# andreaskoepf/faster-rcnn.torch

Hardware: AMD Instinct MI355X
Metric: images/sec (vgg_small 800x450 fwd+bwd) (higher is better)
Workload: dtype f32 (conv / Linear(13824,1024) operands as 2 x fp16 split planes: 22 significand bits, 3 MFMA partial products; fp32 accumulate)

## Files before the change

### faster-rcnn.torch_amd/csrc/conv.hip

```cpp
#include <cstdlib>

#include "kernels.h"
#include "amax.h"
#include <type_traits>

namespace frcnn {

typedef float f32x16 __attribute__((ext_vector_type(16)));

int conv_cc(int k) { return k == 1 ? 32 : (k == 3 ? 8 : 2); }
int conv_mpad(int M) { return M <= 64 ? 64 : cdiv(M, 128) * 128; }
size_t conv_pack_floats(int Kchan, int M, int k) {
  int cc = conv_cc(k);
  return (size_t)cdiv(Kchan, cc) * cc * k * k * conv_mpad(M);
}

__global__ void pack_weights_kernel(const float* __restrict__ w, int O, int C, int k, int mode,
                                    int Kchan_pad, int M, int Mpad, float* __restrict__ dst) {
  long total = (long)Kchan_pad * k * k * Mpad;
  for (long t = (long)blockIdx.x * blockDim.x + threadIdx.x; t < total;
       t += (long)gridDim.x * blockDim.x) {
    int m = (int)(t % Mpad);
    long row = t / Mpad;
    int h = (int)(row & 1);
// ... 1198 lines not shown
  hipLaunchKernelGGL(wgrad_reduce_map_kernel, dim3(rgrid), dim3(256), 0, s, slab, nSplit, taps, O, C, gw, map);
  return FRCNN_OK;
}

size_t conv_wgrad_workspace_bytes(int Cin, int H, int W, int O, int k, int pad) {
  if (k == 3 && Cin % 64 == 0 && O % 64 == 0) {
    WgradArgs b;
    b.Cin = Cin; b.H = H; b.W = W; b.O = O; b.pad = pad; b.Ho = H + 2 * pad - k + 1; b.Wo = W + 2 * pad - k + 1;
    wgrad_plan(b, k);
    return std::max((size_t)b.nSplit * k * k * O * Cin * 4 + 256, conv_wgradx_workspace_bytes(Cin, H, W, O, pad));
  }
  WgradArgs a;
  a.Cin = Cin; a.H = H; a.W = W; a.O = O; a.pad = pad;
  a.Ho = H + 2 * pad - k + 1; a.Wo = W + 2 * pad - k + 1;
  wgrad_plan(a, k);
  return (size_t)a.nSplit * (k * k * O * Cin + O + 1) * 4 + 256;
}

template <int KS, int TYS, int PM>
static int launch_wgrad_pm(WgradArgs& a, int klass, double flops, float* gw, hipStream_t s) {
  size_t lds = ((size_t)64 * WG_NTP + (size_t)64 * (PM == 2 ? 129 : WG_PP)) * 4;
  static bool attr_set = false;
  if (!attr_set) {
    FR_HIP(hipFuncSetAttribute(reinterpret_cast<const void*>(conv_wgrad_kernel<KS, TYS, PM>),
                               hipFuncAttributeMaxDynamicSharedMemorySize, 160 * 1024));
    attr_set = true;
  }
  int grid = a.oTiles * a.cTiles * a.kyGroups * a.nSplit;
  double bytes = 4.0 * ((double)a.Cin * a.H * a.W + (double)a.O * a.Ho * a.Wo);
  if (frcnn::prof_enabled(klass)) frcnn::prof_before(klass, s);
  hipLaunchKernelGGL((conv_wgrad_kernel<KS, TYS, PM>), dim3(grid), dim3(256), lds, s, a);
// ... 99 lines not shown
```

### faster-rcnn.torch_amd/csrc/net.cpp

```cpp
#include <array>
#include <vector>
#include <cmath>
#include <cstring>

#include "kernels.h"

namespace frcnn {

static const int HEAD_OUT = 18;
static const int SPARSE_MAX_POS = 512;

struct DevBuf {
  void* p = nullptr;
  size_t bytes = 0;
  bool owned = true;
  void view(void* ptr, size_t n) { p = ptr; bytes = n; owned = false; }
  int ensure(size_t need) {
    if (need <= bytes) return FRCNN_OK;
    if (p && owned) (void)hipFree(p);
    owned = true;
    p = nullptr; bytes = 0;
    FR_HIP(hipMalloc(&p, need + 64));
    bytes = need;
    return FRCNN_OK;
// ... 13 lines not shown
  DevBuf x, gx;
  int am = -1;
};

struct Block {
  int first_conv, nconv;
  bool has_drop;
  float p_drop;
  DevBuf scale;
  DevBuf pooled, gpooled;
  DevBuf pidx;
  int Hp, Wp;
  int am = -1;
  bool dc_on = false;
  int nk = 0, nkM = 0, nkK = 0;
  const int* dc_idx = nullptr;
  DevBuf dc_bias;
};

struct Head {
  Conv c3;
  Conv c1;
  int input;
  DevBuf delta;
  const int* sp_pos = nullptr;
  int sp_count = -1;
  DevBuf spD, spHX, spHY, spGH, spCol, spDX;
  DevBuf spOut, spSlab;
  hipStream_t stream = nullptr;
  hipEvent_t done = nullptr;
// ... 11 lines not shown
  DevBuf xp, xpT, gp, gpT;
  int x_form = 0;
  DevBuf am;
  const float* am_w_of = nullptr;
  long am_w_gen = -1;
};

}

using namespace frcnn;

static int g_drop_compact = -1;
static int drop_compact_on() {
  if (g_drop_compact < 0) g_drop_compact = getenv("FRCNN_DROP_COMPACT") ? (atoi(getenv("FRCNN_DROP_COMPACT")) != 0) : 1;
  return g_drop_compact;
}
static int pool_stream(int slot, hipStream_t* out) {
  static hipStream_t pool[8] = {};
  if (!pool[slot]) FR_HIP(hipStreamCreateWithFlags(&pool[slot], hipStreamNonBlocking));
  *out = pool[slot];
  return FRCNN_OK;
}

static int g_sparse_heads = -1;
static int sparse_heads_on() {
  if (g_sparse_heads < 0) g_sparse_heads = getenv("FRCNN_SPARSE_HEADS") ? (atoi(getenv("FRCNN_SPARSE_HEADS")) != 0) : 1;
  return g_sparse_heads;
}
static int g_static_weights = 0;
static long g_static_gen = 0;
// ... 550 lines not shown
int frcnn_model_update_join(frcnn_model* m, void* stream) {
  FR_CHECK(m != nullptr, "model_update_join: null model");
  FR_TRY(ensure_update_stream(m));
  FR_HIP(hipEventRecord(m->upd_join_ev, m->cw));
  FR_HIP(hipStreamWaitEvent(S(stream), m->upd_join_ev, 0));
  return FRCNN_OK;
}

int frcnn_get_option(const char* name, int* value) {
  FR_CHECK(name != nullptr && value != nullptr, "get_option: null argument");
  if (strcmp(name, "side_stream") == 0) { *value = side_enabled() ? 1 : 0; return FRCNN_OK; }
  if (strcmp(name, "gemm_x_roles") == 0) { *value = get_gemm_x_roles(); return FRCNN_OK; }
  if (strcmp(name, "deterministic") == 0) { *value = deterministic() ? 1 : 0; return FRCNN_OK; }
  if (strcmp(name, "static_weights") == 0) { *value = g_static_weights; return FRCNN_OK; }
  if (strcmp(name, "drop_compact") == 0) { *value = drop_compact_on(); return FRCNN_OK; }
  if (strcmp(name, "sparse_heads") == 0) { *value = sparse_heads_on(); return FRCNN_OK; }
  if (strcmp(name, "winograd") == 0) { *value = 0; return FRCNN_OK; }
  if (strcmp(name, "cnet_wgrad_async") == 0) { *value = g_cnet_wgrad_async; return FRCNN_OK; }
  if (strcmp(name, "split_bf16") == 0) { *value = get_split_bf16(); return FRCNN_OK; }
  if (strcmp(name, "x3_f16") == 0) { *value = get_x3_f16(); return FRCNN_OK; }
  FR_CHECK(false, "get_option: unknown option '%s'", name);
  return FRCNN_OK;
}

int frcnn_set_option(const char* name, int value) {
  FR_CHECK(name != nullptr, "set_option: null name");
  if (strcmp(name, "side_stream") == 0) { g_side_stream = value ? 1 : 0; return FRCNN_OK; }
  if (strcmp(name, "deterministic") == 0) { set_deterministic(value != 0); return FRCNN_OK; }
  if (strcmp(name, "static_weights") == 0) { g_static_weights = value != 0; ++g_static_gen; return FRCNN_OK; }
  if (strcmp(name, "drop_compact") == 0) { g_drop_compact = value != 0; return FRCNN_OK; }
  if (strcmp(name, "sparse_heads") == 0) { g_sparse_heads = value != 0; return FRCNN_OK; }
  if (strcmp(name, "gemm_x_roles") == 0) { set_gemm_x_roles(value); return FRCNN_OK; }
  if (strcmp(name, "split_bf16") == 0) { set_split_bf16(value); return FRCNN_OK; }
  if (strcmp(name, "x3_f16") == 0) { set_x3_f16(value); return FRCNN_OK; }
  if (strcmp(name, "winograd") == 0) return FRCNN_OK;
  if (strcmp(name, "cnet_wgrad_async") == 0) { g_cnet_wgrad_async = value ? 1 : 0; return FRCNN_OK; }
  FR_CHECK(false, "set_option: unknown option '%s'", name);
  return FRCNN_OK;
}

static int ensure_head_streams(frcnn_model* m);
static int ensure_side(frcnn_model* m) {
  if (!m->side) {
    FR_TRY(pool_stream(0, &m->side));
    FR_HIP(hipEventCreateWithFlags(&m->join_ev, hipEventDisableTiming));
// ... 111 lines not shown
      for (int i = 0; i < C; ++i) keep[i] = frcnn_keep_mask(seed * 131 + b, (unsigned long long)i, blk.p_drop);
    }
    int nk = 0;
    bool binary = true;
    for (int i = 0; i < C; ++i) {
      if (keep[i] == 1.0f) idx_host[my + nk++] = i;
      else if (keep[i] != 0.0f) binary = false;
    }
    if (!binary) continue;
    for (int i = nk; i < C; ++i) idx_host[my + i] = -1;
    const int nkM = std::min(C, (nk + 63) / 64 * 64), nkK = std::min(C, (nk + 15) / 16 * 16);
    if (nk == 0 || nkK >= C) continue;
    if (!conv_x3_eligible(c0.Cin, nkM, 3) || !conv_x3_eligible(nkK, c1.Cout, 3) || !conv_x3_eligible(c1.Cout, nkM, 3) ||
        (b > 0 && !conv_x3_eligible(nkK, c0.Cin, 3)) || !conv_wgradx_eligible(nkM, c1.Cout, 3) || !conv_wgradx_eligible(c0.Cin, nkM, 3))
      continue;
    blk.dc_on = true; blk.nk = nk; blk.nkM = nkM; blk.nkK = nkK; blk.dc_idx = idx_dev + my;
  }
  return FRCNN_OK;
}

static int pack_compact(frcnn_model* m, const float* w, bool f16, hipStream_t s) {
  const unsigned slot = m->dc_step % frcnn_model::DC_RING;
  ++m->dc_step;
  char* hslot = m->dc_pin + (size_t)slot * m->dc_slot_bytes;
  char* dslot = (char*)m->dc_dev.p + (size_t)slot * m->dc_slot_bytes;
  const std::vector<PackXJob>& src = f16 ? m->x3_host16 : m->x3_host;
  PackXJob* jobs = (PackXJob*)hslot;
  int n = 0;
  for (int i = 0; i < (int)src.size(); ++i) {
    PackXJob j = src[i];
    const int ci = m->x3_conv[i];
// ... 687 lines not shown
                            grad + c.b_off, grad + c.a_off, s, (c.x_d && m->f16_packed) ? m->rec(c.am + 1) : nullptr));
      }
      const float* in; const float* in_slope = nullptr; const float* in_scale = nullptr;
      if (st > 0) {
        Conv& pc = m->convs[blk.first_conv + st - 1];
        in = pc.x.f(); in_slope = w + pc.a_off;
        in_scale = (st - 1 == 0 && blk.has_drop) ? blk.scale.f() : nullptr;
      } else {
        in = b == 0 ? m->img.f() : m->blocks[b - 1].pooled.f();
      }
      const bool dc = blk.dc_on && st <= 1;
      int wg_cin = c.Cin, wg_o = c.Cout;
      WgradMap wmap;
      if (dc) {
        wmap.Cfull = c.Cin;
        if (st == 1) { wg_cin = blk.nkM; wmap.cmap = blk.dc_idx; in_scale = nullptr; }
        else { wg_o = blk.nkM; wmap.omap = blk.dc_idx; }
      }
      const float* wa_in = nullptr; const float* wa_g = nullptr;
      if (m->f16_packed && c.x_f && c.x_d && (st > 0 || b > 0)) {
        wa_in = st > 0 ? m->rec(m->convs[blk.first_conv + st - 1].am) : m->rec(m->blocks[b - 1].am);
        wa_g = m->rec(c.am + 1);
      }
      const bool on_caller = use_side && b == 0 && st == 0;
      if (use_side && !on_caller) FR_TRY(fork_side(m, s, n_fork++));
      if (on_caller) {
        FR_TRY(conv_wgrad(in, wg_cin, c.H, c.W, in_slope, in_scale, c.gx.f(), wg_o, c.k, c.pad, grad + c.w_off, m->wg_ws_first.p,
                          m->wg_ws_first.bytes, s, fused_here ? grad + c.b_off : nullptr, wa_in, wa_g, dc ? &wmap : nullptr));
        FR_HIP(hipEventRecord(m->join_ev, ws));
        FR_HIP(hipStreamWaitEvent(s, m->join_ev, 0));
      } else {
// ... 287 lines not shown
```

### faster-rcnn.torch_amd/csrc/wgradx.hip

```cpp
#include <cstdlib>

#include "kernels.h"
#include "amax.h"
#include <type_traits>

namespace frcnn {

typedef float f32x16 __attribute__((ext_vector_type(16)));
typedef __bf16 bf16x8 __attribute__((ext_vector_type(8)));
typedef __bf16 bf16x4 __attribute__((ext_vector_type(4)));
typedef __bf16 bf16x2 __attribute__((ext_vector_type(2)));
typedef float f32x2 __attribute__((ext_vector_type(2)));
typedef _Float16 f16x8 __attribute__((ext_vector_type(8)));
typedef _Float16 f16x2 __attribute__((ext_vector_type(2)));

#define WX_TH 4
#define WX_TW 16
#define WX_GROW 128
#define WX_GPLANE (64 * WX_GROW)
#define WX_XROW 48
#define WX_XCH (6 * WX_XROW)
#define WX_XPLANE (64 * WX_XCH + 8 * 16)
#define WX_LDS (3 * WX_GPLANE + 3 * WX_XPLANE)

bool conv_wgradx_eligible(int Cin, int O, int k) {
  return get_split_bf16() && k == 3 && Cin % 64 == 0 && O % 64 == 0;
}

__device__ __forceinline__ unsigned wx_cvt2(float a, float b) {
  f32x2 v = {a, b};
  bf16x2 r = __builtin_convertvector(v, bf16x2);
  return __builtin_bit_cast(unsigned, r);
}
__device__ __forceinline__ void wx_split4(const float* v, uint2& H, uint2& Mi, uint2& L) {
  unsigned h[2], m[2], l[2];
#pragma unroll
  for (int j = 0; j < 2; ++j) {
    const float x0 = v[2 * j], x1 = v[2 * j + 1];
    h[j] = wx_cvt2(x0, x1);
    const float r0 = x0 - __builtin_bit_cast(float, h[j] << 16), r1 = x1 - __builtin_bit_cast(float, h[j] & 0xFFFF0000u);
    m[j] = wx_cvt2(r0, r1);
// ... 16 lines not shown
}
__device__ __forceinline__ float wx_pow2(int e) { return __builtin_bit_cast(float, (unsigned)(e + 127) << 23); }

struct WgradXArgs {
  const float* in;
  const float* in_slope;
  const float* in_scale;
  const float* g;
  float* slab;
  float* gbias;
  const float* amax_in;
  const float* amax_g;
  const int* omap;
  int Cin, H, W, O, Ho, Wo, pad;
  int tilesX, tilesY, oTiles, cTiles, nSplit;
};

__device__ __forceinline__ unsigned wx_xaddr(int c) { return (unsigned)(c * WX_XCH + (c >> 3) * 16); }
__device__ __forceinline__ unsigned wx_gswz(int o) { const unsigned u = (o >> 1) & 7; return ((u & 3) << 1) | (u >> 2); }

typedef unsigned u32x4 __attribute__((ext_vector_type(4)));
typedef float f32x4u __attribute__((ext_vector_type(4), aligned(4)));

#define WX_PIN(x) asm volatile("" : "+v"(x))

template <int N, class F>
__device__ __forceinline__ void static_for(F&& f) {
  if constexpr (N > 0) {
    static_for<N - 1>(f);
    f(std::integral_constant<int, N - 1>{});
  }
}

template <bool SLOPE, bool SCALE, int VEC, int NP = 3>
__global__ __launch_bounds__(256, 1) void conv_wgradx_kernel(WgradXArgs p) {
  extern __shared__ __attribute__((aligned(16))) char smem[];
  constexpr unsigned LDSI = NP * (WX_GPLANE + WX_XPLANE), XB = NP * WX_GPLANE;
  const int tid = threadIdx.x, lane = tid & 63;
  const int wave = __builtin_amdgcn_readfirstlane(tid >> 6);
  const int wo = wave >> 1, wc = wave & 1;
  const int h = lane >> 5, li = lane & 31;

  int bid;
  {
    const int nblk = gridDim.x, xcd = blockIdx.x & 7, idx = blockIdx.x >> 3;
    const int q = nblk >> 3, r = nblk & 7;
    bid = xcd * q + min(xcd, r) + idx;
  }
  const int ot = bid % p.oTiles; bid /= p.oTiles;
  const int ct = bid % p.cTiles;
  const int split = bid / p.cTiles;
  const int o0 = ot * 64, c0 = ct * 64;
  const int HW = p.H * p.W, HoWo = p.Ho * p.Wo;
  const float slope = SLOPE ? *p.in_slope : 1.f;
  float gmul = 1.f, xmul = 1.f, out_mul = 1.f, out_mul2 = 1.f;
  if (NP == 2) {
    const float ag = amax_load_block(p.amax_g);
    float ax = amax_load_block(p.amax_in);
    if (SLOPE) ax *= fmaxf(1.f, fabsf(slope));
    const int eg = wx_exp(ag, 14), ex = wx_exp(ax, SCALE ? 13 : 14);
    gmul = wx_pow2(eg); xmul = wx_pow2(ex);
    const int et = -(eg + ex), e1 = et / 2;
    out_mul = wx_pow2(e1); out_mul2 = wx_pow2(et - e1);
  }

  f32x16 acc[9];
#pragma unroll
  for (int t = 0; t < 9; ++t)
#pragma unroll
    for (int r = 0; r < 16; ++r) acc[t][r] = 0.f;

  const int srow = tid >> 2, sq = tid & 3;
  const float* const gsrc = p.g + (size_t)(o0 + srow) * HoWo;
  const float* const xsrc = p.in + (size_t)(c0 + srow) * HW;
  auto gat = [&](int elem_off) { return gsrc + elem_off; };
  auto xat = [&](int elem_off) { return xsrc + elem_off; };
  const float xscale = SCALE ? p.in_scale[c0 + srow] : 1.f;
  const unsigned gdst = (unsigned)(srow * WX_GROW) + ((((unsigned)sq >> 1) ^ wx_gswz(srow)) << 4) + (sq & 1) * 8;
  const unsigned xdst = XB + wx_xaddr(srow) + sq * 8;
  int xr[9], xs[9];
#pragma unroll
  for (int k = 0; k < 9; ++k) {
    const int j = sq + 4 * k;
    xr[k] = j / 6; xs[k] = j - 6 * xr[k];
  }

  const int oA = wo * 32 + li, cB = wc * 32 + li;
  const unsigned abase = (unsigned)(oA * WX_GROW) + (((unsigned)h ^ wx_gswz(oA)) << 4);
  const unsigned bbase = XB + wx_xaddr(cB) + h * 16;

  const int nPix = p.tilesX * p.tilesY;
  const int nT = (nPix - split + p.nSplit - 1) / p.nSplit;
  struct Pre {
    float vg[4][4], vx[9][4];
    bool ok[13];
    int oy0, ox0;
  };
#ifdef WX_ONE_SET
  Pre pre[1];
#else
  Pre pre[2];
#endif
  float sr[13][4];
  unsigned sh[13][2], sm[13][2], sl[13][2];
  float bsum = 0.f;
  bool bsum_on = true;
  auto up_lo = [](unsigned v) { return __builtin_bit_cast(float, v << 16); };
  auto up_hi = [](unsigned v) { return __builtin_bit_cast(float, v & 0xFFFF0000u); };
  const int adv_y = p.nSplit / p.tilesX, adv_x = p.nSplit % p.tilesX;
  int w_ty = split / p.tilesX, w_tx = split % p.tilesX, w_i = 0;
  auto load_origin = [&](Pre& P) {
    P.oy0 = w_ty * WX_TH; P.ox0 = w_tx * WX_TW;
    const int more = w_i + 1 < nT ? 1 : 0;
    w_tx += more * adv_x; w_ty += more * adv_y;
    const int wrap = w_tx >= p.tilesX ? 1 : 0;
    w_tx -= wrap * p.tilesX; w_ty += wrap;
    ++w_i;
  };
  auto load_step = [&](auto itc, Pre& P) {
    constexpr int it = decltype(itc)::value;
    const int oy0 = P.oy0, ox0 = P.ox0;
    if constexpr (it < 4) {
      constexpr int k = it;
      const int oy = oy0 + k, ox = ox0 + 4 * sq;
      if (VEC) {
        P.ok[it] = oy < p.Ho && ox < p.Wo;
        const f32x4u v = *reinterpret_cast<const f32x4u*>(gat((oy * p.Wo + ox) & -(int)P.ok[it]));
        P.vg[k][0] = v[0]; P.vg[k][1] = v[1]; P.vg[k][2] = v[2]; P.vg[k][3] = v[3];
      } else {
#pragma unroll
        for (int e = 0; e < 4; ++e) P.vg[k][e] = *gat((oy * p.Wo + ox + e) & -(int)(oy < p.Ho && ox + e < p.Wo));
      }
    } else {
      constexpr int k = it - 4;
      const int iy = oy0 - p.pad + xr[k], ix = ox0 - p.pad - 3 + 4 * xs[k];
      if (VEC) {
        P.ok[it] = (unsigned)iy < (unsigned)p.H && (unsigned)ix < (unsigned)p.W;
        const f32x4u v = *reinterpret_cast<const f32x4u*>(xat((iy * p.W + ix) & -(int)P.ok[it]));
        P.vx[k][0] = v[0]; P.vx[k][1] = v[1]; P.vx[k][2] = v[2]; P.vx[k][3] = v[3];
      } else {
#pragma unroll
        for (int e = 0; e < 4; ++e)
          P.vx[k][e] = *xat((iy * p.W + ix + e) & -(int)((unsigned)iy < (unsigned)p.H && (unsigned)(ix + e) < (unsigned)p.W));
      }
    }
  };
  auto inside = [&](auto itc, int e, Pre& P) -> bool {
    constexpr int it = decltype(itc)::value;
    if (VEC == 1) return P.ok[it];
    if (VEC == 2) {
      if constexpr (it < 4) return P.ok[it] && P.ox0 + 4 * sq + e < p.Wo;
      else return P.ok[it] && P.ox0 - p.pad - 3 + 4 * xs[it < 4 ? 0 : it - 4] + e < p.W;
    }
    if constexpr (it < 4) return P.oy0 + it < p.Ho && P.ox0 + 4 * sq + e < p.Wo;
    else return (unsigned)(P.oy0 - p.pad + xr[it < 4 ? 0 : it - 4]) < (unsigned)p.H &&
                (unsigned)(P.ox0 - p.pad - 3 + 4 * xs[it < 4 ? 0 : it - 4] + e) < (unsigned)p.W;
  };
  constexpr int XPH0 = (SLOPE || SCALE) ? 0 : 4;
  auto stage_step = [&](auto itc, auto phc, unsigned gwb, unsigned xwb, Pre& P) {
    constexpr int it = decltype(itc)::value, ph = decltype(phc)::value;
    if constexpr (ph < 4) {
      constexpr int k = it - 4;
      {
        constexpr int e = ph;
        float v = P.vx[k][e];
        if (SLOPE) v = v > 0.f ? v : slope * v;
        if (SCALE) v *= xscale;
        P.vx[k][e] = inside(itc, e, P) ? v : 0.f;
        WX_PIN(P.vx[k][e]);
      }
    } else if constexpr (ph == 4 || ph == 6) {
      constexpr int j = (ph - 4) / 2;
      float x0 = it < 4 ? P.vg[it < 4 ? it : 0][2 * j] : P.vx[it < 4 ? 0 : it - 4][2 * j];
      float x1 = it < 4 ? P.vg[it < 4 ? it : 0][2 * j + 1] : P.vx[it < 4 ? 0 : it - 4][2 * j + 1];
      if (it < 4 || XPH0 == 4) {
        x0 = inside(itc, 2 * j, P) ? x0 : 0.f;
        x1 = inside(itc, 2 * j + 1, P) ? x1 : 0.f;
      }
      if (it < 4) bsum += bsum_on ? x0 + x1 : 0.f;
      if constexpr (NP == 2) {
        const float mul = it < 4 ? gmul : xmul;
        x0 *= mul; x1 *= mul;
        sh[it][j] = wx_cvt2h(x0, x1);
        const f16x2 hv = __builtin_bit_cast(f16x2, sh[it][j]);
        sr[it][2 * j] = x0 - (float)hv[0];
        sr[it][2 * j + 1] = x1 - (float)hv[1];
      } else {
        sh[it][j] = wx_cvt2(x0, x1);
        sr[it][2 * j] = x0 - up_lo(sh[it][j]);
        sr[it][2 * j + 1] = x1 - up_hi(sh[it][j]);
      }
      WX_PIN(sh[it][j]); WX_PIN(sr[it][2 * j]); WX_PIN(sr[it][2 * j + 1]);
    } else if constexpr (ph == 5 || ph == 7) {
      constexpr int j = (ph - 5) / 2;
      if constexpr (NP == 2) {
        sl[it][j] = wx_cvt2h(sr[it][2 * j], sr[it][2 * j + 1]);
        WX_PIN(sl[it][j]);
      } else {
        sm[it][j] = wx_cvt2(sr[it][2 * j], sr[it][2 * j + 1]);
        const float s0 = sr[it][2 * j] - up_lo(sm[it][j]), s1 = sr[it][2 * j + 1] - up_hi(sm[it][j]);
        sl[it][j] = wx_cvt2(s0, s1);
        WX_PIN(sm[it][j]); WX_PIN(sl[it][j]);
      }
    } else {
      char* d = it < 4 ? smem + (gwb ^ ((unsigned)it << 5)) : smem + xwb + 32 * (it - 4);
      constexpr int PL = it < 4 ? WX_GPLANE : WX_XPLANE;
      *reinterpret_cast<uint2*>(d) = make_uint2(sh[it][0], sh[it][1]);
      if constexpr (NP == 2) {
        *reinterpret_cast<uint2*>(d + PL) = make_uint2(sl[it][0], sl[it][1]);
      } else {
        *reinterpret_cast<uint2*>(d + PL) = make_uint2(sm[it][0], sm[it][1]);
        *reinterpret_cast<uint2*>(d + 2 * PL) = make_uint2(sl[it][0], sl[it][1]);
      }
      asm volatile("" ::: "memory");
    }
  };
  auto stage_seq = [&](auto i0c, auto sc, unsigned gwb, unsigned xwb, Pre& P) {
    constexpr int I0 = decltype(i0c)::value, s = decltype(sc)::value;
    constexpr int NG = I0 < 4 ? 4 - I0 : 0;
    constexpr int NPX = 9 - XPH0;
    constexpr int it = s < 5 * NG ? I0 + s / 5 : I0 + NG + (s - 5 * NG) / NPX;
    constexpr int ph = s < 5 * NG ? 4 + s % 5 : XPH0 + (s - 5 * NG) % NPX;
    stage_step(std::integral_constant<int, it>{}, std::integral_constant<int, ph>{}, gwb, xwb, P);
  };

  u32x4 a[WX_TH][NP];
  u32x4 b[3][NP], bn[3][NP];
  u32x4 raw[NP][2];
  constexpr int NQ = NP == 2 ? 3 : 6;
  constexpr int PA[6] = {NP == 2 ? 1 : 2, 0, NP == 2 ? 0 : 1, 1, 0, 0}, PB[6] = {0, NP == 2 ? 1 : 2, NP == 2 ? 0 : 1, 0, 1, 0};
  auto read_row = [&](unsigned rb, int r) {
    if (r < WX_TH) {
#pragma unroll
      for (int pl = 0; pl < NP; ++pl)
        a[r][pl] = *reinterpret_cast<const u32x4*>(smem + rb + pl * WX_GPLANE + (abase ^ ((unsigned)r << 5)));
    }
#pragma unroll
    for (int pl = 0; pl < NP; ++pl) {
      raw[pl][0] = *reinterpret_cast<const u32x4*>(smem + rb + bbase + pl * WX_XPLANE + r * WX_XROW);
      raw[pl][1] = *reinterpret_cast<const u32x4*>(smem + rb + bbase + pl * WX_XPLANE + r * WX_XROW + 16);
    }
  };
  auto cut_step = [&](auto sc) {
    constexpr int pl = decltype(sc)::value >> 1, hf = decltype(sc)::value & 1;
    const u32x4 d0 = raw[pl][0], d1 = raw[pl][1];
    const unsigned d[8] = {d0[0], d0[1], d0[2], d0[3], d1[0], d1[1], d1[2], d1[3]};
    if (hf == 1) asm volatile("" ::"v"(d[0]), "v"(d[7]));
#pragma unroll
    for (int j = 2 * hf; j < 2 * hf + 2; ++j) {
      bn[0][pl][j] = __builtin_amdgcn_alignbit(d[j + 2], d[j + 1], 16);
      bn[1][pl][j] = d[j + 2];
      bn[2][pl][j] = __builtin_amdgcn_alignbit(d[j + 3], d[j + 2], 16);
      WX_PIN(bn[0][pl][j]); WX_PIN(bn[1][pl][j]); WX_PIN(bn[2][pl][j]);
    }
  };

  load_origin(pre[0]);
  static_for<13>([&](auto itc) { load_step(itc, pre[0]); });
  constexpr int NST = 4 * 5 + 9 * (9 - XPH0);
  static_for<NST>([&](auto sc) { stage_seq(std::integral_constant<int, 0>{}, sc, gdst, xdst, pre[0]); });
  __syncthreads();
#ifdef WX_ONE_SET
  load_origin(pre[0]);
  static_for<13>([&](auto itc) { load_step(itc, pre[0]); });
#else
  load_origin(pre[1]);
  static_for<13>([&](auto itc) { load_step(itc, pre[1]); });
  load_origin(pre[0]);
  static_for<13>([&](auto itc) { load_step(itc, pre[0]); });
#endif
  read_row(0, 0);
  static_for<2 * NP>([&](auto sc) { cut_step(sc); });
#pragma unroll
  for (int kx = 0; kx < 3; ++kx)
#pragma unroll
    for (int pl = 0; pl < NP; ++pl) b[kx][pl] = bn[kx][pl];

  auto tile = [&](int i, Pre& P) {
    const unsigned rb = (i & 1) ? LDSI : 0, wb = LDSI - rb;
    const unsigned gwb = gdst + wb, xwb = xdst + wb;
    bsum_on = i + 1 < nT;
    auto row = [&](auto rc) {
      constexpr int r = decltype(rc)::value;
      constexpr int nky = r < 3 ? r + 1 : 6 - r;
      constexpr int NM = 3 * NQ * nky;
      constexpr int NPX = 9 - XPH0;
      constexpr int NSTG = r == 1 ? 4 * 5 + NPX : (r == 2 || r == 3) ? 4 * NPX : r == 4 ? 13 : 0;
      constexpr int NS = NSTG + 2 * NP;
      __builtin_amdgcn_sched_barrier(0);
      if (r < 5) read_row(rb, r + 1); else read_row(wb, 0);
      __builtin_amdgcn_sched_barrier(0);
      static_for<NM>([&](auto mc) {
        constexpr int m = decltype(mc)::value;
        constexpr int q = m / (3 * nky), kyi = (m / 3) % nky, kx = m % 3;
        constexpr int ky = (r < WX_TH ? 0 : r - (WX_TH - 1)) + kyi, ks = r - ky;
        static_assert(ks >= 0 && ks < WX_TH && ky < 3, "tap walk");
        if constexpr (NP == 2)
          acc[3 * ky + kx] = __builtin_amdgcn_mfma_f32_32x32x16_f16(__builtin_bit_cast(f16x8, a[ks][PA[q]]), __builtin_bit_cast(f16x8, b[kx][PB[q]]), acc[3 * ky + kx], 0, 0, 0);
        else
          acc[3 * ky + kx] = __builtin_amdgcn_mfma_f32_32x32x16_bf16(__builtin_bit_cast(bf16x8, a[ks][PA[q]]), __builtin_bit_cast(bf16x8, b[kx][PB[q]]), acc[3 * ky + kx], 0, 0, 0);
        __builtin_amdgcn_sched_barrier(0);
        constexpr int LEAD = NSTG == 0 ? 6 : 0;
        constexpr int s0 = m < LEAD ? 0 : (m - LEAD) * NS / (NM - LEAD), s1 = m < LEAD ? 0 : (m - LEAD + 1) * NS / (NM - LEAD);
        static_for<s1 - s0>([&](auto dc) {
          constexpr int s = s0 + decltype(dc)::value;
          if constexpr (s >= NSTG) {
            cut_step(std::integral_constant<int, s - NSTG>{});
          } else if constexpr (r >= 1 && r <= 3) {
            stage_seq(std::integral_constant<int, r == 1 ? 0 : r == 2 ? 5 : 9>{}, std::integral_constant<int, s>{}, gwb, xwb, P);
          } else {
            if constexpr (s == 0) load_origin(P);
            load_step(std::integral_constant<int, s>{}, P);
          }
        });
        __builtin_amdgcn_sched_barrier(0);
      });
#pragma unroll
      for (int kx = 0; kx < 3; ++kx)
#pragma unroll
        for (int pl = 0; pl < NP; ++pl) b[kx][pl] = bn[kx][pl];
      if (r == 4) __syncthreads();
    };
    row(std::integral_constant<int, 0>{}); row(std::integral_constant<int, 1>{}); row(std::integral_constant<int, 2>{});
    row(std::integral_constant<int, 3>{}); row(std::integral_constant<int, 4>{}); row(std::integral_constant<int, 5>{});
  };
  {
    int i = 0;
#ifdef WX_ONE_SET
    for (; i < nT; ++i) tile(i, pre[0]);
#else
    for (; i + 1 < nT; i += 2) { tile(i, pre[1]); tile(i + 1, pre[0]); }
    if (i < nT) tile(i, pre[1]);
#endif
  }
  if (p.gbias && ct == 0) {
    float v = bsum;
    v += __shfl_xor(v, 1); v += __shfl_xor(v, 2);
    const int od = p.omap ? p.omap[o0 + srow] : o0 + srow;
    if (sq == 0 && od >= 0) unsafeAtomicAdd(p.gbias + od, v);
  }
  {
    const int c = c0 + wc * 32 + li;
    const size_t OC = (size_t)p.O * p.Cin;
    float* sl = p.slab + (size_t)split * 9 * OC;
#pragma unroll
    for (int tap = 0; tap < 9; ++tap)
#pragma unroll
      for (int r = 0; r < 16; ++r) {
        const int o = o0 + wo * 32 + (r & 3) + 8 * (r >> 2) + 4 * h;
        sl[(size_t)tap * OC + (size_t)o * p.Cin + c] = NP == 2 ? (acc[tap][r] * out_mul) * out_mul2 : acc[tap][r];
      }
  }
}

static void wgradx_plan(WgradXArgs& a) {
  a.tilesX = cdiv(a.Wo, WX_TW); a.tilesY = cdiv(a.Ho, WX_TH);
  a.oTiles = a.O / 64; a.cTiles = a.Cin / 64;
  const long base = (long)a.oTiles * a.cTiles, npix = (long)a.tilesX * a.tilesY;
  a.nSplit = (int)std::max<long>(1, std::min<long>(npix, 256 / base));
  if (const char* e = getenv("FRCNN_WGX_NSPLIT")) a.nSplit = (int)std::max<long>(1, std::min<long>(npix, atoi(e)));
}

size_t conv_wgradx_workspace_bytes(int Cin, int H, int W, int O, int pad) {
  WgradXArgs a;
  a.Cin = Cin; a.H = H; a.W = W; a.O = O; a.pad = pad; a.Ho = H + 2 * pad - 2; a.Wo = W + 2 * pad - 2;
  wgradx_plan(a);
  return (size_t)a.nSplit * 9 * O * Cin * 4 + 256;
}

static const WgradMap* g_wx_map = nullptr;

template <bool SLOPE, bool SCALE, int VEC, int NP = 3>
static int launch_wgradx_v(WgradXArgs& a, double flops, float* gw, hipStream_t s) {
  static bool attr_set = false;
  if (!attr_set) {
    FR_HIP(hipFuncSetAttribute(reinterpret_cast<const void*>(conv_wgradx_kernel<SLOPE, SCALE, VEC, NP>),
                               hipFuncAttributeMaxDynamicSharedMemorySize, NP == 2 ? 120 * 1024 : 160 * 1024));
    attr_set = true;
  }
  const int grid = a.oTiles * a.cTiles * a.nSplit;
  const double bytes = 4.0 * ((double)a.Cin * a.H * a.W + (double)a.O * a.Ho * a.Wo);
  if (prof_enabled(KC_CONV_WGRADX)) prof_before(KC_CONV_WGRADX, s);
  const size_t lds = 2 * (size_t)NP * (WX_GPLANE + WX_XPLANE);
  hipLaunchKernelGGL((conv_wgradx_kernel<SLOPE, SCALE, VEC, NP>), dim3(grid), dim3(256), lds, s, a);
  if (g_wx_map) FR_TRY(wgrad_reduce_map(a.slab, a.nSplit, 9, a.O, a.Cin, gw, *g_wx_map, s));
  else FR_TRY(wgrad_reduce(a.slab, a.nSplit, 9, a.O * a.Cin, gw, s));
  if (prof_enabled(KC_CONV_WGRADX)) prof_after(KC_CONV_WGRADX, flops, bytes, s);
  FR_LAUNCH_CHECK();
  return FRCNN_OK;
}

static bool readable_past_end(const void* p, size_t bytes, size_t slack) {
  hipDeviceptr_t base = nullptr;
  size_t size = 0;
  if (hipMemGetAddressRange(&base, &size, (hipDeviceptr_t)p) != hipSuccess) { (void)hipGetLastError(); return false; }
  return (uintptr_t)p + bytes + slack <= (uintptr_t)base + size;
}

template <bool SLOPE, bool SCALE, int NP = 3>
static int launch_wgradx(WgradXArgs& a, double flops, float* gw, hipStream_t s) {
  if (a.pad == 1 && a.W % 4 == 0 && ((uintptr_t)a.in & 15) == 0 && ((uintptr_t)a.g & 15) == 0)
    return launch_wgradx_v<SLOPE, SCALE, 1, NP>(a, flops, gw, s);
  if (a.pad == 1 && readable_past_end(a.in, (size_t)a.Cin * a.H * a.W * 4, 12) && readable_past_end(a.g, (size_t)a.O * a.Ho * a.Wo * 4, 12))
    return launch_wgradx_v<SLOPE, SCALE, 2, NP>(a, flops, gw, s);
  return launch_wgradx_v<SLOPE, SCALE, 0, NP>(a, flops, gw, s);
}

int conv_wgradx(const float* in, int Cin, int H, int W, const float* in_slope, const float* in_scale, const float* g, int O,
                int pad, float* gw, void* ws, size_t ws_bytes, hipStream_t s, float* gbias, const float* amax_in, const float* amax_g,
                const WgradMap* map) {
  WgradXArgs a;
  a.in = in; a.in_slope = in_slope; a.in_scale = in_scale; a.g = g; a.gbias = gbias;
  a.amax_in = amax_in; a.amax_g = amax_g;
  a.omap = map ? map->omap : nullptr;
  struct MapScope { MapScope(const WgradMap* m) { g_wx_map = (m && (m->omap || m->cmap)) ? m : nullptr; } ~MapScope() { g_wx_map = nullptr; } } scope(map);
  FR_CHECK((amax_in != nullptr) == (amax_g != nullptr), "conv_wgradx: the fp16 form needs the magnitude records of both tensors");
  a.Cin = Cin; a.H = H; a.W = W; a.O = O; a.pad = pad; a.Ho = H + 2 * pad - 2; a.Wo = W + 2 * pad - 2;
  FR_CHECK(Cin % 64 == 0 && O % 64 == 0, "conv_wgradx: %d channels x %d filters is not a split-bf16 shape", Cin, O);
  FR_CHECK((long)Cin * H * W < (1L << 30) && (long)O * a.Ho * a.Wo < (1L << 30), "conv_wgradx: tensor too large for 32-bit offsets");
  wgradx_plan(a);
  const size_t need = (size_t)a.nSplit * 9 * O * Cin * 4 + 256;
  FR_CHECK(ws && ws_bytes >= need, "conv_wgradx: workspace too small (%zu < %zu)", ws_bytes, need);
  a.slab = (float*)(((uintptr_t)ws + 255) / 256 * 256);
  const double flops = 2.0 * O * Cin * 9 * (double)a.Ho * a.Wo;
  if (amax_in) {
    if (in_slope) return in_scale ? launch_wgradx<true, true, 2>(a, flops, gw, s) : launch_wgradx<true, false, 2>(a, flops, gw, s);
    return in_scale ? launch_wgradx<false, true, 2>(a, flops, gw, s) : launch_wgradx<false, false, 2>(a, flops, gw, s);
  }
  if (in_slope) return in_scale ? launch_wgradx<true, true>(a, flops, gw, s) : launch_wgradx<true, false>(a, flops, gw, s);
  return in_scale ? launch_wgradx<false, true>(a, flops, gw, s) : launch_wgradx<false, false>(a, flops, gw, s);
}

}
// ... 1 lines not shown
```

Baseline: 512.4.

## Add 128x32 wgradx block shape and round dropout-compacted channels to 32

Adds a second tile shape (128 filters x 32 channels, four waves along O) to the split-precision weight-gradient kernel, so channel counts that are multiples of 32 but not 64 become eligible. The dropout-compacted block now rounds its kept-channel count up to a configurable granularity (32 by default) instead of the 64-based padded count for the wgrad input side, so less padded work is done. The change costs more template instantiations, new LDS layout arithmetic, and a possibly less efficient tile shape for the narrow-channel case.

```diff
diff --git a/faster-rcnn.torch_amd/csrc/conv.hip b/faster-rcnn.torch_amd/csrc/conv.hip
--- a/faster-rcnn.torch_amd/csrc/conv.hip
+++ b/faster-rcnn.torch_amd/csrc/conv.hip
@@ -1236,7 +1236,8 @@
   a.Cin = Cin; a.H = H; a.W = W; a.O = O; a.pad = pad;
   a.Ho = H + 2 * pad - k + 1; a.Wo = W + 2 * pad - k + 1;
   wgrad_plan(a, k);
-  return (size_t)a.nSplit * (k * k * O * Cin + O + 1) * 4 + 256;
+  const size_t fp32 = (size_t)a.nSplit * (k * k * O * Cin + O + 1) * 4 + 256;
+  return k == 3 && Cin % 32 == 0 && O % 128 == 0 ? std::max(fp32, conv_wgradx_workspace_bytes(Cin, H, W, O, pad)) : fp32;
 }
 
 template <int KS, int TYS, int PM>
diff --git a/faster-rcnn.torch_amd/csrc/net.cpp b/faster-rcnn.torch_amd/csrc/net.cpp
--- a/faster-rcnn.torch_amd/csrc/net.cpp
+++ b/faster-rcnn.torch_amd/csrc/net.cpp
@@ -51,6 +51,7 @@
   int am = -1;
   bool dc_on = false;
   int nk = 0, nkM = 0, nkK = 0;
+  int nkW = 0;
   const int* dc_idx = nullptr;
   DevBuf dc_bias;
 };
@@ -92,6 +93,12 @@
 static int drop_compact_on() {
   if (g_drop_compact < 0) g_drop_compact = getenv("FRCNN_DROP_COMPACT") ? (atoi(getenv("FRCNN_DROP_COMPACT")) != 0) : 1;
   return g_drop_compact;
+}
+static int g_drop_gran = -1;
+static int drop_compact_gran() {
+  if (g_drop_gran < 0) g_drop_gran = getenv("FRCNN_DROP_COMPACT_GRAN") ? atoi(getenv("FRCNN_DROP_COMPACT_GRAN")) : 32;
+  if (g_drop_gran != 32 && g_drop_gran != 64) g_drop_gran = 32;
+  return g_drop_gran;
 }
 static int pool_stream(int slot, hipStream_t* out) {
   static hipStream_t pool[8] = {};
@@ -672,6 +679,7 @@
   if (strcmp(name, "deterministic") == 0) { *value = deterministic() ? 1 : 0; return FRCNN_OK; }
   if (strcmp(name, "static_weights") == 0) { *value = g_static_weights; return FRCNN_OK; }
   if (strcmp(name, "drop_compact") == 0) { *value = drop_compact_on(); return FRCNN_OK; }
+  if (strcmp(name, "drop_compact_gran") == 0) { *value = drop_compact_gran(); return FRCNN_OK; }
   if (strcmp(name, "sparse_heads") == 0) { *value = sparse_heads_on(); return FRCNN_OK; }
   if (strcmp(name, "winograd") == 0) { *value = 0; return FRCNN_OK; }
   if (strcmp(name, "cnet_wgrad_async") == 0) { *value = g_cnet_wgrad_async; return FRCNN_OK; }
@@ -687,6 +695,10 @@
   if (strcmp(name, "deterministic") == 0) { set_deterministic(value != 0); return FRCNN_OK; }
   if (strcmp(name, "static_weights") == 0) { g_static_weights = value != 0; ++g_static_gen; return FRCNN_OK; }
   if (strcmp(name, "drop_compact") == 0) { g_drop_compact = value != 0; return FRCNN_OK; }
+  if (strcmp(name, "drop_compact_gran") == 0) {
+    FR_CHECK(value == 32 || value == 64, "set_option: drop_compact_gran is 32 or 64, not %d", value);
+    g_drop_gran = value; return FRCNN_OK;
+  }
   if (strcmp(name, "sparse_heads") == 0) { g_sparse_heads = value != 0; return FRCNN_OK; }
   if (strcmp(name, "gemm_x_roles") == 0) { set_gemm_x_roles(value); return FRCNN_OK; }
   if (strcmp(name, "split_bf16") == 0) { set_split_bf16(value); return FRCNN_OK; }
@@ -828,7 +840,9 @@
     if (!conv_x3_eligible(c0.Cin, nkM, 3) || !conv_x3_eligible(nkK, c1.Cout, 3) || !conv_x3_eligible(c1.Cout, nkM, 3) ||
         (b > 0 && !conv_x3_eligible(nkK, c0.Cin, 3)) || !conv_wgradx_eligible(nkM, c1.Cout, 3) || !conv_wgradx_eligible(c0.Cin, nkM, 3))
       continue;
-    blk.dc_on = true; blk.nk = nk; blk.nkM = nkM; blk.nkK = nkK; blk.dc_idx = idx_dev + my;
+    const int gran = drop_compact_gran(), nkG = std::min(nkM, (nk + gran - 1) / gran * gran);
+    const int nkW = conv_wgradx_eligible(nkG, c1.Cout, 3) ? nkG : nkM;
+    blk.dc_on = true; blk.nk = nk; blk.nkM = nkM; blk.nkK = nkK; blk.nkW = nkW; blk.dc_idx = idx_dev + my;
   }
   return FRCNN_OK;
 }
@@ -1546,7 +1560,7 @@
       WgradMap wmap;
       if (dc) {
         wmap.Cfull = c.Cin;
-        if (st == 1) { wg_cin = blk.nkM; wmap.cmap = blk.dc_idx; in_scale = nullptr; }
+        if (st == 1) { wg_cin = blk.nkW; wmap.cmap = blk.dc_idx; in_scale = nullptr; }
         else { wg_o = blk.nkM; wmap.omap = blk.dc_idx; }
       }
       const float* wa_in = nullptr; const float* wa_g = nullptr;
diff --git a/faster-rcnn.torch_amd/csrc/wgradx.hip b/faster-rcnn.torch_amd/csrc/wgradx.hip
--- a/faster-rcnn.torch_amd/csrc/wgradx.hip
+++ b/faster-rcnn.torch_amd/csrc/wgradx.hip
@@ -22,9 +22,13 @@
 #define WX_XCH (6 * WX_XROW)
 #define WX_XPLANE (64 * WX_XCH + 8 * 16)
 #define WX_LDS (3 * WX_GPLANE + 3 * WX_XPLANE)
+constexpr unsigned wx_gplane(int ow) { return (unsigned)(32 * ow) * WX_GROW; }
+constexpr unsigned wx_xplane(int ow) { return ((unsigned)(128 / ow) * WX_XCH + (unsigned)(128 / ow / 8) * 16 + 127) / 128 * 128; }
+static_assert(wx_gplane(2) == WX_GPLANE && wx_xplane(2) == WX_XPLANE, "the 64 x 64 block's LDS layout");
+static int wx_ow(int Cin, int O) { return Cin % 64 == 0 && O % 64 == 0 ? 2 : 4; }
 
 bool conv_wgradx_eligible(int Cin, int O, int k) {
-  return get_split_bf16() && k == 3 && Cin % 64 == 0 && O % 64 == 0;
+  return get_split_bf16() && k == 3 && ((Cin % 64 == 0 && O % 64 == 0) || (Cin % 32 == 0 && O % 128 == 0));
 }
 
 __device__ __forceinline__ unsigned wx_cvt2(float a, float b) {
@@ -71,6 +75,7 @@
   const int* omap;
   int Cin, H, W, O, Ho, Wo, pad;
   int tilesX, tilesY, oTiles, cTiles, nSplit;
+  int ow;
 };
 
 __device__ __forceinline__ unsigned wx_xaddr(int c) { return (unsigned)(c * WX_XCH + (c >> 3) * 16); }
@@ -89,13 +94,17 @@
   }
 }
 
-template <bool SLOPE, bool SCALE, int VEC, int NP = 3>
+template <bool SLOPE, bool SCALE, int VEC, int NP = 3, int OW = 2>
 __global__ __launch_bounds__(256, 1) void conv_wgradx_kernel(WgradXArgs p) {
   extern __shared__ __attribute__((aligned(16))) char smem[];
-  constexpr unsigned LDSI = NP * (WX_GPLANE + WX_XPLANE), XB = NP * WX_GPLANE;
+  constexpr unsigned GPL = wx_gplane(OW), XPL = wx_xplane(OW);
+  constexpr unsigned LDSI = NP * (GPL + XPL), XB = NP * GPL;
+  constexpr int BO = 32 * OW, BC = 128 / OW;
+  constexpr int NGI = BO / 16, NXI = (BC * 36 + 255) / 256;
+  static_assert(NGI + NXI == 13 && (OW == 2 || OW == 4), "block shape");
   const int tid = threadIdx.x, lane = tid & 63;
   const int wave = __builtin_amdgcn_readfirstlane(tid >> 6);
-  const int wo = wave >> 1, wc = wave & 1;
+  const int wo = OW == 2 ? wave >> 1 : wave, wc = OW == 2 ? wave & 1 : 0;
   const int h = lane >> 5, li = lane & 31;
 
   int bid;
@@ -107,7 +116,7 @@
   const int ot = bid % p.oTiles; bid /= p.oTiles;
   const int ct = bid % p.cTiles;
   const int split = bid / p.cTiles;
-  const int o0 = ot * 64, c0 = ct * 64;
+  const int o0 = ot * BO, c0 = ct * BC;
   const int HW = p.H * p.W, HoWo = p.Ho * p.Wo;
   const float slope = SLOPE ? *p.in_slope : 1.f;
   float gmul = 1.f, xmul = 1.f, out_mul = 1.f, out_mul2 = 1.f;
@@ -127,19 +136,26 @@
 #pragma unroll
     for (int r = 0; r < 16; ++r) acc[t][r] = 0.f;
 
-  const int srow = tid >> 2, sq = tid & 3;
-  const float* const gsrc = p.g + (size_t)(o0 + srow) * HoWo;
-  const float* const xsrc = p.in + (size_t)(c0 + srow) * HW;
+  const int grow = OW == 2 ? tid >> 2 : tid >> 1, gq = OW == 2 ? tid & 3 : tid & 1;
+  const int xrow = OW == 2 ? tid >> 2 : tid >> 3, xq = OW == 2 ? tid & 3 : tid & 7;
+  const int gcol = 4 * gq;
+  auto g_row = [](int k) { return OW == 2 ? k : k >> 1; };
+  auto g_cx = [](int k) { return OW == 2 ? 0 : 8 * (k & 1); };
+  const float* const gsrc = p.g + (size_t)(o0 + grow) * HoWo;
+  const float* const xsrc = p.in + (size_t)(c0 + xrow) * HW;
   auto gat = [&](int elem_off) { return gsrc + elem_off; };
   auto xat = [&](int elem_off) { return xsrc + elem_off; };
-  const float xscale = SCALE ? p.in_scale[c0 + srow] : 1.f;
-  const unsigned gdst = (unsigned)(srow * WX_GROW) + ((((unsigned)sq >> 1) ^ wx_gswz(srow)) << 4) + (sq & 1) * 8;
-  const unsigned xdst = XB + wx_xaddr(srow) + sq * 8;
-  int xr[9], xs[9];
-#pragma unroll
-  for (int k = 0; k < 9; ++k) {
-    const int j = sq + 4 * k;
+  const float xscale = SCALE ? p.in_scale[c0 + xrow] : 1.f;
+  const unsigned gdst = OW == 2 ? (unsigned)(grow * WX_GROW) + ((((unsigned)gq >> 1) ^ wx_gswz(grow)) << 4) + (gq & 1) * 8
+                                : (unsigned)(grow * WX_GROW) + (wx_gswz(grow) << 4) + gq * 8;
+  const unsigned xdst = XB + wx_xaddr(xrow) + (OW == 2 ? xq * 8 : 0);
+  int xr[NXI], xs[NXI];
+  unsigned xo[NXI];
+#pragma unroll
+  for (int k = 0; k < NXI; ++k) {
+    const int j = OW == 2 ? xq + 4 * k : min(xq + 8 * k, 35);
     xr[k] = j / 6; xs[k] = j - 6 * xr[k];
+    xo[k] = 8 * j;
   }
 
   const int oA = wo * 32 + li, cB = wc * 32 + li;
@@ -149,7 +165,7 @@
   const int nPix = p.tilesX * p.tilesY;
   const int nT = (nPix - split + p.nSplit - 1) / p.nSplit;
   struct Pre {
-    float vg[4][4], vx[9][4];
+    float vg[NGI][4], vx[NXI][4];
     bool ok[13];
     int oy0, ox0;
   };
@@ -177,9 +193,9 @@
   auto load_step = [&](auto itc, Pre& P) {
     constexpr int it = decltype(itc)::value;
     const int oy0 = P.oy0, ox0 = P.ox0;
-    if constexpr (it < 4) {
+    if constexpr (it < NGI) {
       constexpr int k = it;
-      const int oy = oy0 + k, ox = ox0 + 4 * sq;
+      const int oy = oy0 + g_row(k), ox = ox0 + gcol + g_cx(k);
       if (VEC) {
         P.ok[it] = oy < p.Ho && ox < p.Wo;
         const f32x4u v = *reinterpret_cast<const f32x4u*>(gat((oy * p.Wo + ox) & -(int)P.ok[it]));
@@ -189,7 +205,7 @@
         for (int e = 0; e < 4; ++e) P.vg[k][e] = *gat((oy * p.Wo + ox + e) & -(int)(oy < p.Ho && ox + e < p.Wo));
       }
     } else {
-      constexpr int k = it - 4;
+      constexpr int k = it - NGI;
       const int iy = oy0 - p.pad + xr[k], ix = ox0 - p.pad - 3 + 4 * xs[k];
       if (VEC) {
         P.ok[it] = (unsigned)iy < (unsigned)p.H && (unsigned)ix < (unsigned)p.W;
@@ -206,18 +222,18 @@
     constexpr int it = decltype(itc)::value;
     if (VEC == 1) return P.ok[it];
     if (VEC == 2) {
-      if constexpr (it < 4) return P.ok[it] && P.ox0 + 4 * sq + e < p.Wo;
-      else return P.ok[it] && P.ox0 - p.pad - 3 + 4 * xs[it < 4 ? 0 : it - 4] + e < p.W;
+      if constexpr (it < NGI) return P.ok[it] && P.ox0 + gcol + g_cx(it) + e < p.Wo;
+      else return P.ok[it] && P.ox0 - p.pad - 3 + 4 * xs[it < NGI ? 0 : it - NGI] + e < p.W;
     }
-    if constexpr (it < 4) return P.oy0 + it < p.Ho && P.ox0 + 4 * sq + e < p.Wo;
-    else return (unsigned)(P.oy0 - p.pad + xr[it < 4 ? 0 : it - 4]) < (unsigned)p.H &&
-                (unsigned)(P.ox0 - p.pad - 3 + 4 * xs[it < 4 ? 0 : it - 4] + e) < (unsigned)p.W;
+    if constexpr (it < NGI) return P.oy0 + g_row(it) < p.Ho && P.ox0 + gcol + g_cx(it) + e < p.Wo;
+    else return (unsigned)(P.oy0 - p.pad + xr[it < NGI ? 0 : it - NGI]) < (unsigned)p.H &&
+                (unsigned)(P.ox0 - p.pad - 3 + 4 * xs[it < NGI ? 0 : it - NGI] + e) < (unsigned)p.W;
   };
   constexpr int XPH0 = (SLOPE || SCALE) ? 0 : 4;
   auto stage_step = [&](auto itc, auto phc, unsigned gwb, unsigned xwb, Pre& P) {
     constexpr int it = decltype(itc)::value, ph = decltype(phc)::value;
     if constexpr (ph < 4) {
-      constexpr int k = it - 4;
+      constexpr int k = it - NGI;
       {
         constexpr int e = ph;
         float v = P.vx[k][e];
@@ -228,15 +244,15 @@
       }
     } else if constexpr (ph == 4 || ph == 6) {
       constexpr int j = (ph - 4) / 2;
-      float x0 = it < 4 ? P.vg[it < 4 ? it : 0][2 * j] : P.vx[it < 4 ? 0 : it - 4][2 * j];
-      float x1 = it < 4 ? P.vg[it < 4 ? it : 0][2 * j + 1] : P.vx[it < 4 ? 0 : it - 4][2 * j + 1];
-      if (it < 4 || XPH0 == 4) {
+      float x0 = it < NGI ? P.vg[it < NGI ? it : 0][2 * j] : P.vx[it < NGI ? 0 : it - NGI][2 * j];
+      float x1 = it < NGI ? P.vg[it < NGI ? it : 0][2 * j + 1] : P.vx[it < NGI ? 0 : it - NGI][2 * j + 1];
+      if (it < NGI || XPH0 == 4) {
         x0 = inside(itc, 2 * j, P) ? x0 : 0.f;
         x1 = inside(itc, 2 * j + 1, P) ? x1 : 0.f;
       }
-      if (it < 4) bsum += bsum_on ? x0 + x1 : 0.f;
+      if (it < NGI) bsum += bsum_on ? x0 + x1 : 0.f;
       if constexpr (NP == 2) {
-        const float mul = it < 4 ? gmul : xmul;
+        const float mul = it < NGI ? gmul : xmul;
         x0 *= mul; x1 *= mul;
         sh[it][j] = wx_cvt2h(x0, x1);
         const f16x2 hv = __builtin_bit_cast(f16x2, sh[it][j]);
@@ -260,8 +276,9 @@
         WX_PIN(sm[it][j]); WX_PIN(sl[it][j]);
       }
     } else {
-      char* d = it < 4 ? smem + (gwb ^ ((unsigned)it << 5)) : smem + xwb + 32 * (it - 4);
-      constexpr int PL = it < 4 ? WX_GPLANE : WX_XPLANE;
+      char* d = it < NGI ? smem + (gwb ^ ((unsigned)it << (OW == 2 ? 5 : 4)))
+                         : smem + xwb + (OW == 2 ? 32u * (it - NGI) : xo[it < NGI ? 0 : it - NGI]);
+      constexpr int PL = it < NGI ? GPL : XPL;
       *reinterpret_cast<uint2*>(d) = make_uint2(sh[it][0], sh[it][1]);
       if constexpr (NP == 2) {
         *reinterpret_cast<uint2*>(d + PL) = make_uint2(sl[it][0], sl[it][1]);
@@ -272,9 +289,9 @@
       asm volatile("" ::: "memory");
     }
   };
-  auto stage_seq = [&](auto i0c, auto sc, unsigned gwb, unsigned xwb, Pre& P) {
-    constexpr int I0 = decltype(i0c)::value, s = decltype(sc)::value;
-    constexpr int NG = I0 < 4 ? 4 - I0 : 0;
+  auto stage_seq = [&](auto i0c, auto i1c, auto sc, unsigned gwb, unsigned xwb, Pre& P) {
+    constexpr int I0 = decltype(i0c)::value, I1 = decltype(i1c)::value, s = decltype(sc)::value;
+    constexpr int NG = I0 < NGI ? (I1 < NGI ? I1 : NGI) - I0 : 0;
     constexpr int NPX = 9 - XPH0;
     constexpr int it = s < 5 * NG ? I0 + s / 5 : I0 + NG + (s - 5 * NG) / NPX;
     constexpr int ph = s < 5 * NG ? 4 + s % 5 : XPH0 + (s - 5 * NG) % NPX;
@@ -290,12 +307,12 @@
     if (r < WX_TH) {
 #pragma unroll
       for (int pl = 0; pl < NP; ++pl)
-        a[r][pl] = *reinterpret_cast<const u32x4*>(smem + rb + pl * WX_GPLANE + (abase ^ ((unsigned)r << 5)));
+        a[r][pl] = *reinterpret_cast<const u32x4*>(smem + rb + pl * GPL + (abase ^ ((unsigned)r << 5)));
     }
 #pragma unroll
     for (int pl = 0; pl < NP; ++pl) {
-      raw[pl][0] = *reinterpret_cast<const u32x4*>(smem + rb + bbase + pl * WX_XPLANE + r * WX_XROW);
-      raw[pl][1] = *reinterpret_cast<const u32x4*>(smem + rb + bbase + pl * WX_XPLANE + r * WX_XROW + 16);
+      raw[pl][0] = *reinterpret_cast<const u32x4*>(smem + rb + bbase + pl * XPL + r * WX_XROW);
+      raw[pl][1] = *reinterpret_cast<const u32x4*>(smem + rb + bbase + pl * XPL + r * WX_XROW + 16);
     }
   };
   auto cut_step = [&](auto sc) {
@@ -314,8 +331,8 @@
 
   load_origin(pre[0]);
   static_for<13>([&](auto itc) { load_step(itc, pre[0]); });
-  constexpr int NST = 4 * 5 + 9 * (9 - XPH0);
-  static_for<NST>([&](auto sc) { stage_seq(std::integral_constant<int, 0>{}, sc, gdst, xdst, pre[0]); });
+  constexpr int NST = NGI * 5 + NXI * (9 - XPH0);
+  static_for<NST>([&](auto sc) { stage_seq(std::integral_constant<int, 0>{}, std::integral_constant<int, 13>{}, sc, gdst, xdst, pre[0]); });
   __syncthreads();
 #ifdef WX_ONE_SET
   load_origin(pre[0]);
@@ -342,7 +359,9 @@
       constexpr int nky = r < 3 ? r + 1 : 6 - r;
       constexpr int NM = 3 * NQ * nky;
       constexpr int NPX = 9 - XPH0;
-      constexpr int NSTG = r == 1 ? 4 * 5 + NPX : (r == 2 || r == 3) ? 4 * NPX : r == 4 ? 13 : 0;
+      constexpr int I0 = r == 1 ? 0 : r == 2 ? 5 : 9, I1 = r == 1 ? 5 : r == 2 ? 9 : 13;
+      constexpr int NGR = I0 < NGI ? (I1 < NGI ? I1 : NGI) - I0 : 0;
+      constexpr int NSTG = (r >= 1 && r <= 3) ? 5 * NGR + NPX * (I1 - I0 - NGR) : r == 4 ? 13 : 0;
       constexpr int NS = NSTG + 2 * NP;
       __builtin_amdgcn_sched_barrier(0);
       if (r < 5) read_row(rb, r + 1); else read_row(wb, 0);
@@ -364,7 +383,7 @@
           if constexpr (s >= NSTG) {
             cut_step(std::integral_constant<int, s - NSTG>{});
           } else if constexpr (r >= 1 && r <= 3) {
-            stage_seq(std::integral_constant<int, r == 1 ? 0 : r == 2 ? 5 : 9>{}, std::integral_constant<int, s>{}, gwb, xwb, P);
+            stage_seq(std::integral_constant<int, I0>{}, std::integral_constant<int, I1>{}, std::integral_constant<int, s>{}, gwb, xwb, P);
           } else {
             if constexpr (s == 0) load_origin(P);
             load_step(std::integral_constant<int, s>{}, P);
@@ -392,9 +411,10 @@
   }
   if (p.gbias && ct == 0) {
     float v = bsum;
-    v += __shfl_xor(v, 1); v += __shfl_xor(v, 2);
-    const int od = p.omap ? p.omap[o0 + srow] : o0 + srow;
-    if (sq == 0 && od >= 0) unsafeAtomicAdd(p.gbias + od, v);
+    v += __shfl_xor(v, 1);
+    if (OW == 2) v += __shfl_xor(v, 2);
+    const int od = p.omap ? p.omap[o0 + grow] : o0 + grow;
+    if (gq == 0 && od >= 0) unsafeAtomicAdd(p.gbias + od, v);
   }
   {
     const int c = c0 + wc * 32 + li;
@@ -412,7 +432,8 @@
 
 static void wgradx_plan(WgradXArgs& a) {
   a.tilesX = cdiv(a.Wo, WX_TW); a.tilesY = cdiv(a.Ho, WX_TH);
-  a.oTiles = a.O / 64; a.cTiles = a.Cin / 64;
+  a.ow = wx_ow(a.Cin, a.O);
+  a.oTiles = a.O / (32 * a.ow); a.cTiles = a.Cin / (128 / a.ow);
   const long base = (long)a.oTiles * a.cTiles, npix = (long)a.tilesX * a.tilesY;
   a.nSplit = (int)std::max<long>(1, std::min<long>(npix, 256 / base));
   if (const char* e = getenv("FRCNN_WGX_NSPLIT")) a.nSplit = (int)std::max<long>(1, std::min<long>(npix, atoi(e)));
@@ -427,19 +448,19 @@
 
 static const WgradMap* g_wx_map = nullptr;
 
-template <bool SLOPE, bool SCALE, int VEC, int NP = 3>
+template <bool SLOPE, bool SCALE, int VEC, int NP = 3, int OW = 2>
 static int launch_wgradx_v(WgradXArgs& a, double flops, float* gw, hipStream_t s) {
   static bool attr_set = false;
   if (!attr_set) {
-    FR_HIP(hipFuncSetAttribute(reinterpret_cast<const void*>(conv_wgradx_kernel<SLOPE, SCALE, VEC, NP>),
+    FR_HIP(hipFuncSetAttribute(reinterpret_cast<const void*>(conv_wgradx_kernel<SLOPE, SCALE, VEC, NP, OW>),
                                hipFuncAttributeMaxDynamicSharedMemorySize, NP == 2 ? 120 * 1024 : 160 * 1024));
     attr_set = true;
   }
   const int grid = a.oTiles * a.cTiles * a.nSplit;
   const double bytes = 4.0 * ((double)a.Cin * a.H * a.W + (double)a.O * a.Ho * a.Wo);
   if (prof_enabled(KC_CONV_WGRADX)) prof_before(KC_CONV_WGRADX, s);
-  const size_t lds = 2 * (size_t)NP * (WX_GPLANE + WX_XPLANE);
-  hipLaunchKernelGGL((conv_wgradx_kernel<SLOPE, SCALE, VEC, NP>), dim3(grid), dim3(256), lds, s, a);
+  const size_t lds = 2 * (size_t)NP * (wx_gplane(OW) + wx_xplane(OW));
+  hipLaunchKernelGGL((conv_wgradx_kernel<SLOPE, SCALE, VEC, NP, OW>), dim3(grid), dim3(256), lds, s, a);
   if (g_wx_map) FR_TRY(wgrad_reduce_map(a.slab, a.nSplit, 9, a.O, a.Cin, gw, *g_wx_map, s));
   else FR_TRY(wgrad_reduce(a.slab, a.nSplit, 9, a.O * a.Cin, gw, s));
   if (prof_enabled(KC_CONV_WGRADX)) prof_after(KC_CONV_WGRADX, flops, bytes, s);
@@ -454,13 +475,17 @@
   return (uintptr_t)p + bytes + slack <= (uintptr_t)base + size;
 }
 
+template <bool SLOPE, bool SCALE, int NP = 3, int OW = 2>
+static int launch_wgradx_s(WgradXArgs& a, double flops, float* gw, hipStream_t s) {
+  if (a.pad == 1 && a.W % 4 == 0 && ((uintptr_t)a.in & 15) == 0 && ((uintptr_t)a.g & 15) == 0)
+    return launch_wgradx_v<SLOPE, SCALE, 1, NP, OW>(a, flops, gw, s);
+  if (a.pad == 1 && readable_past_end(a.in, (size_t)a.Cin * a.H * a.W * 4, 12) && readable_past_end(a.g, (size_t)a.O * a.Ho * a.Wo * 4, 12))
+    return launch_wgradx_v<SLOPE, SCALE, 2, NP, OW>(a, flops, gw, s);
+  return launch_wgradx_v<SLOPE, SCALE, 0, NP, OW>(a, flops, gw, s);
+}
 template <bool SLOPE, bool SCALE, int NP = 3>
 static int launch_wgradx(WgradXArgs& a, double flops, float* gw, hipStream_t s) {
-  if (a.pad == 1 && a.W % 4 == 0 && ((uintptr_t)a.in & 15) == 0 && ((uintptr_t)a.g & 15) == 0)
-    return launch_wgradx_v<SLOPE, SCALE, 1, NP>(a, flops, gw, s);
-  if (a.pad == 1 && readable_past_end(a.in, (size_t)a.Cin * a.H * a.W * 4, 12) && readable_past_end(a.g, (size_t)a.O * a.Ho * a.Wo * 4, 12))
-    return launch_wgradx_v<SLOPE, SCALE, 2, NP>(a, flops, gw, s);
-  return launch_wgradx_v<SLOPE, SCALE, 0, NP>(a, flops, gw, s);
+  return a.ow == 2 ? launch_wgradx_s<SLOPE, SCALE, NP, 2>(a, flops, gw, s) : launch_wgradx_s<SLOPE, SCALE, NP, 4>(a, flops, gw, s);
 }
 
 int conv_wgradx(const float* in, int Cin, int H, int W, const float* in_slope, const float* in_scale, const float* g, int O,
@@ -473,7 +498,7 @@
   struct MapScope { MapScope(const WgradMap* m) { g_wx_map = (m && (m->omap || m->cmap)) ? m : nullptr; } ~MapScope() { g_wx_map = nullptr; } } scope(map);
   FR_CHECK((amax_in != nullptr) == (amax_g != nullptr), "conv_wgradx: the fp16 form needs the magnitude records of both tensors");
   a.Cin = Cin; a.H = H; a.W = W; a.O = O; a.pad = pad; a.Ho = H + 2 * pad - 2; a.Wo = W + 2 * pad - 2;
-  FR_CHECK(Cin % 64 == 0 && O % 64 == 0, "conv_wgradx: %d channels x %d filters is not a split-bf16 shape", Cin, O);
+  FR_CHECK((Cin % 64 == 0 && O % 64 == 0) || (Cin % 32 == 0 && O % 128 == 0), "conv_wgradx: %d channels x %d filters is not a split-bf16 shape", Cin, O);
   FR_CHECK((long)Cin * H * W < (1L << 30) && (long)O * a.Ho * a.Wo < (1L << 30), "conv_wgradx: tensor too large for 32-bit offsets");
   wgradx_plan(a);
   const size_t need = (size_t)a.nSplit * 9 * O * Cin * 4 + 256;
```

New measurement: 521.7, median of 6. 1.02x the previous value.
